# huyhoang17/DB_text_minimal

Hardware: AMD Instinct MI355X
Metric: train images/sec @640x640 bs=16/GPU (higher is better)
Workload: dtype f32

## Files before the change

### db_text_minimal_amd/csrc/winograd_wgrad_f32.hip

```cpp
#include "igemm_common.h"
#include <algorithm>

namespace {

constexpr int WG_XPX = 180, WG_XROW = 18, WG_YPX = 128, WG_YROW = 16;

struct WinoWgradParams {
    const float* x;
    const float* dy;
    float* slab;
    int N, H, W, Cx, Cy;
    int nob, nib;
    int tw, gpi, groups;
    int nsplit;
    unsigned x_bytes, dy_bytes;
    const float *x_scale, *x_shift;
};

constexpr int WL_XPX = 336, WL_YPX = 240;
template <bool LIN>
__global__ __launch_bounds__(512) __attribute__((amdgpu_waves_per_eu(2, 2))) void winograd_wgrad_f32_kernel(const WinoWgradParams p) {
    constexpr int XPX = LIN ? WL_XPX : WG_XPX, YPX = LIN ? WL_YPX : WG_YPX;
    constexpr int XCH = XPX * 16, YCH = YPX * 16;
    constexpr int NXP = (XCH + 511) / 512, NYP = (YCH + 511) / 512;
    constexpr int NBUF = LIN ? 1 : 2;
    __shared__ f32x4 smem[NBUF * (XCH + YCH)];
    const int tid = threadIdx.x, lane = tid & 63, wave = __builtin_amdgcn_readfirstlane(tid >> 6);
    const int li = lane & 31, lh = lane >> 5;
    const int irow = wave & 3, oh = wave >> 2;
    const int nsub = p.nob * p.nib;
    const int b = dbn_xcd_remap(blockIdx.x, gridDim.x);
    const int split = b / nsub, sub = b - split * nsub;
    const int ob = sub / p.nib, ib = sub - ob * p.nib;
    const int g0 = (int)((long)split * p.groups / p.nsplit), g1 = (int)((long)(split + 1) * p.groups / p.nsplit);
    const __amdgpu_buffer_rsrc_t rsX = __builtin_amdgcn_make_buffer_rsrc(const_cast<float*>(p.x), 0, p.x_bytes, 0x00020000);
    const __amdgpu_buffer_rsrc_t rsY = __builtin_amdgcn_make_buffer_rsrc(const_cast<float*>(p.dy), 0, p.dy_bytes, 0x00020000);
    const int TW = (p.W + 1) >> 1, TI = ((p.H + 1) >> 1) * TW;
    const int prow = LIN ? 2 * TW + 2 : WG_XROW, yrow = LIN ? 2 * TW : WG_YROW;
    const float rTW = 1.0f / (float)TW;

    unsigned xrel[NXP], yrel[NYP];
    int xpos[NXP], ypos[NYP];
#pragma unroll
    for (int j = 0; j < NXP; ++j) {
        const int idx = tid + j * 512, pix = idx >> 4, ch = idx & 15;
        int py, px;
        if constexpr (LIN) divmod24(pix, prow, 1.0f / (float)prow, py, px);
        else { py = pix / WG_XROW; px = pix - py * WG_XROW; }
        xrel[j] = (unsigned)((py * p.W + px) * p.Cx + ch * 4) * 4u;
        xpos[j] = idx < XCH ? (py | (px << 8)) : -1;
    }
#pragma unroll
    for (int j = 0; j < NYP; ++j) {
        const int idx = tid + j * 512, pix = idx >> 4, ch = idx & 15;
        int py, px;
        if constexpr (LIN) divmod24(pix, yrow, 1.0f / (float)yrow, py, px);
        else { py = pix >> 4; px = pix & 15; }
        yrel[j] = (unsigned)((py * p.W + px) * p.Cy + ch * 4) * 4u;
        ypos[j] = idx < YCH ? (py | (px << 8)) : -1;
    }
    f32x4 rx[NXP], ry[LIN ? 1 : NYP];
    const bool act = p.x_scale != nullptr;
    f32x4 asc_ = {0.f, 0.f, 0.f, 0.f}, ash_ = {0.f, 0.f, 0.f, 0.f};
    if (act && !LIN) {
        asc_ = *reinterpret_cast<const f32x4*>(p.x_scale + ib * 64 + (tid & 15) * 4);
        ash_ = *reinterpret_cast<const f32x4*>(p.x_shift + ib * 64 + (tid & 15) * 4);
    }
    unsigned xstatic = 0;
#pragma unroll
    for (int j = 0; j < NXP; ++j) xstatic |= (unsigned)(xpos[j] >= 0) << j;
    unsigned xvalid = 0;
    int t0 = 0, tr0 = 0;
    auto geometry = [&](int g, int& n, int& hs0, int& ws0, int& xrows) {
        n = g / p.gpi;
        const int t = g - n * p.gpi;
        if constexpr (LIN) {
            const int tfirst = t * 32, tlast = min(tfirst + 31, TI - 1);
            const int r0_ = tfirst / TW, r1_ = tlast / TW;
            hs0 = 2 * r0_ - 1;
            ws0 = -1;
            xrows = 2 * (r1_ - r0_ + 1) + 2;
        } else {
            const int ty = t / p.tw, tx = t - ty * p.tw;
            hs0 = ty * 8 - 1;
            ws0 = tx * 16 - 1;
            xrows = 10;
        }
    };
    auto load_x = [&](int g) {
        int n, hs0, ws0, xrows;
        geometry(g, n, hs0, ws0, xrows);
        const unsigned bx = (unsigned)(((n * p.H + hs0) * p.W + ws0) * p.Cx + ib * 64) * 4u;
        if (!LIN && hs0 >= 0 && hs0 + 10 <= p.H && ws0 >= 0 && ws0 + WG_XROW <= p.W) {
#pragma unroll
            for (int j = 0; j < NXP; ++j) rx[j] = buffer_load_f32x4(rsX, xpos[j] >= 0 ? bx + xrel[j] : OOB_OFFSET);
            xvalid = xstatic;
            return;
        }
#pragma unroll
        for (int j = 0; j < NXP; ++j) {
            const int py = xpos[j] & 255, px = xpos[j] >> 8;
            const bool v = xpos[j] >= 0 && py < xrows && (unsigned)(hs0 + py) < (unsigned)p.H && (unsigned)(ws0 + px) < (unsigned)p.W;
            rx[j] = buffer_load_f32x4(rsX, v ? bx + xrel[j] : OOB_OFFSET);
// ... 100 lines not shown
            float dd[4], D[4];
            auto fetch = [&](int s_) {
                const int xo = xoff2 + (2 * (s_ >> 2) * WG_XROW + 4 * (s_ & 3)) * 32, yo = yoff4 + (2 * (s_ >> 2) * WG_YROW + 4 * (s_ & 3)) * 64;
#pragma unroll
                for (int q = 0; q < 4; ++q) {
                    U1[q] = Xr1[xo + q * 32];
                    U2[q] = Xr2[xo + q * 32];
                }
                dd[0] = Yb[yo];
                dd[1] = Yb[yo + 64];
                dd[2] = Yb[yo + WG_YROW * 64];
                dd[3] = Yb[yo + WG_YROW * 64 + 64];
            };
            auto form = [&]() {
                f32x2 R[4];
#pragma unroll
                for (int q = 0; q < 4; ++q) {
                    R[q][0] = fmaf(sa, U2[q][0], U1[q][0]);
                    R[q][1] = fmaf(sa, U2[q][1], U1[q][1]);
                }
                V[0] = R[0] - R[2];
                V[1] = R[1] + R[2];
                V[2] = R[2] - R[1];
                V[3] = R[1] - R[3];
                const float r0 = fmaf(c1, dd[2], c0 * dd[0]), r1 = fmaf(c1, dd[3], c0 * dd[1]);
                D[0] = r0;
                D[1] = r0 + r1;
                D[2] = r0 - r1;
                D[3] = -r1;
            };
            fetch(0);
            form();
#pragma unroll
            for (int s = 0; s < 16; ++s) {
                f32x2 Vc[4];
                float Dc[4];
#pragma unroll
                for (int j = 0; j < 4; ++j) {
                    Vc[j] = V[j];
                    Dc[j] = D[j];
                }
                __builtin_amdgcn_sched_barrier(0);
                if (s + 1 < 16) fetch(s + 1);
                __builtin_amdgcn_sched_barrier(0);
#pragma unroll
                for (int j = 0; j < 4; ++j)
#pragma unroll
                    for (int h = 0; h < 2; ++h) acc[j][h] = __builtin_amdgcn_mfma_f32_32x32x2f32(Dc[j], Vc[j][h], acc[j][h], 0, 0, 0);
                __builtin_amdgcn_sched_barrier(0);
                if (s + 1 < 16) form();
            }
        } else {
#pragma unroll
            for (int s = 0; s < 16; ++s) {
                const int t = t0 + 2 * s + lh;
                const bool ok = t < TI;
                int ty, tx;
                divmod24(ok ? t : t0, TW, rTW, ty, tx);
                ty -= tr0;
                const int xo = (2 * ty * prow + 2 * tx) * 32, yo = (2 * ty * yrow + 2 * tx) * 64;
                const float c0s = ok ? c0 : 0.f, c1s = ok ? c1 : 0.f;
                f32x2 R[4];
#pragma unroll
                for (int q = 0; q < 4; ++q) {
                    const f32x2 u1 = Xr1[xoff2 + xo + q * 32], u2 = Xr2[xoff2 + xo + q * 32];
                    R[q][0] = fmaf(sa, u2[0], u1[0]);
                    R[q][1] = fmaf(sa, u2[1], u1[1]);
                }
                const float* const Yc = Yb + yoff4;
                const float d00 = Yc[yo], d01 = Yc[yo + 64], d10 = Yc[yo + yrow * 64], d11 = Yc[yo + yrow * 64 + 64];
                const f32x2 V[4] = {R[0] - R[2], R[1] + R[2], R[2] - R[1], R[1] - R[3]};
                const float r0 = fmaf(c1s, d10, c0s * d00), r1 = fmaf(c1s, d11, c0s * d01);
                const float D[4] = {r0, r0 + r1, r0 - r1, -r1};
#pragma unroll
                for (int j = 0; j < 4; ++j)
#pragma unroll
                    for (int h = 0; h < 2; ++h) acc[j][h] = __builtin_amdgcn_mfma_f32_32x32x2f32(D[j], V[j][h], acc[j][h], 0, 0, 0);
            }
        }
        if constexpr (!LIN) {
            if (g + 1 < g1) __syncthreads();
        }
    }
    float* const S = p.slab + ((long)b * 16 + 4 * irow) * 4096 + (oh * 32 + 4 * lh) * 64 + 2 * li;
#pragma unroll
    for (int j = 0; j < 4; ++j)
#pragma unroll
        for (int r = 0; r < 16; ++r) {
            f32x2 v;
            v[0] = acc[j][0][r];
            v[1] = acc[j][1][r];
            *reinterpret_cast<f32x2*>(S + j * 4096 + ((r & 3) + 8 * (r >> 2)) * 64) = v;
        }
}

__global__ __launch_bounds__(1024) void winograd_wgrad_reduce_serial_kernel(const float* __restrict__ slab, int nsplit, int nsub, int nib, int I,
                                                                     float* __restrict__ grad, float scale) {
    __shared__ double sh[16][64];
    __shared__ float st[576];
    const int o = blockIdx.x, ib = blockIdx.y, sub = (o >> 6) * nib + ib;
    const int pnt = threadIdx.x >> 6, il = threadIdx.x & 63;
    const float* src = slab + ((long)sub * 16 + pnt) * 4096 + (o & 63) * 64 + il;
    const long stride = (long)nsub * 16 * 4096;
    double s = 0.0;
    int z = 0;
    for (; z + 3 < nsplit; z += 4)
        s += ((double)src[z * stride] + (double)src[(z + 1) * stride]) + ((double)src[(z + 2) * stride] + (double)src[(z + 3) * stride]);
    for (; z < nsplit; ++z) s += (double)src[z * stride];
    sh[pnt][il] = s;
    __syncthreads();
    if (threadIdx.x < 576) {
        const int c = threadIdx.x / 9, tap = threadIdx.x - c * 9, r = tap / 3, q = tap - r * 3;
        auto gcol = [](int k, double v0, double v1, double v2, double v3) {
            return k == 0 ? v0 + 0.5 * (v1 + v2) : (k == 1 ? 0.5 * (v1 - v2) : 0.5 * (v1 + v2) + v3);
        };
        double t[4];
#pragma unroll
        for (int i = 0; i < 4; ++i) t[i] = gcol(q, sh[4 * i + 0][c], sh[4 * i + 1][c], sh[4 * i + 2][c], sh[4 * i + 3][c]);
        st[threadIdx.x] = (float)(gcol(r, t[0], t[1], t[2], t[3]) * (double)scale);
    }
    __syncthreads();
    const int n = min(64, I - ib * 64) * 9;
    float* dst = grad + ((long)o * I + ib * 64) * 9;
    for (int k = threadIdx.x; k < n; k += 1024) dst[k] = st[k];
}

template <int ZL>
__global__ __launch_bounds__(256) void winograd_wgrad_reduce_kernel(const float* __restrict__ slab, int nsplit, int nsub, int nib, int I,
                                                                    float* __restrict__ grad, float scale) {
    constexpr int OG = 32 / ZL, ZH = ZL / 2;
    __shared__ double part[ZH * OG][16][32 + 1];
    __shared__ double sh[OG][16][32];
    __shared__ float st[OG * 288];
    const int ib = blockIdx.y >> 1, ih = blockIdx.y & 1;
    const int iq = threadIdx.x & 7, og = (threadIdx.x >> 3) % OG, zl2 = threadIdx.x / (8 * OG), zl = zl2 % ZH;
    const int o = blockIdx.x * OG + og, sub = (o >> 6) * nib + ib;
    const float* src = slab + (long)sub * 16 * 4096 + (o & 63) * 64 + ih * 32 + iq * 4;
    const long stride = (long)nsub * 16 * 4096;
    const int z0 = (int)((long)zl2 * nsplit / ZL), z1 = (int)((long)(zl2 + 1) * nsplit / ZL);
    double acc[16][4];
#pragma unroll
    for (int pt = 0; pt < 16; ++pt)
#pragma unroll
        for (int e = 0; e < 4; ++e) acc[pt][e] = 0.0;
    for (int z = z0; z < z1; ++z) {
        f32x4 v[16];
#pragma unroll
        for (int pt = 0; pt < 16; ++pt) v[pt] = *reinterpret_cast<const f32x4*>(src + z * stride + pt * 4096);
#pragma unroll
        for (int pt = 0; pt < 16; ++pt)
#pragma unroll
            for (int e = 0; e < 4; ++e) acc[pt][e] += (double)v[pt][e];
    }
    if (zl2 >= ZH) {
#pragma unroll
        for (int pt = 0; pt < 16; ++pt)
#pragma unroll
            for (int e = 0; e < 4; ++e) part[zl * OG + og][pt][iq * 4 + e] = acc[pt][e];
    }
    __syncthreads();
    if (zl2 < ZH) {
#pragma unroll
        for (int pt = 0; pt < 16; ++pt)
#pragma unroll
            for (int e = 0; e < 4; ++e) part[zl * OG + og][pt][iq * 4 + e] += acc[pt][e];
    }
    __syncthreads();
    for (int k = threadIdx.x; k < OG * 16 * 32; k += 256) {
        const int g = k >> 9, pt = (k >> 5) & 15, c = k & 31;
        double s_ = 0.0;
#pragma unroll
        for (int q = 0; q < ZH; ++q) s_ += part[q * OG + g][pt][c];
        sh[g][pt][c] = s_;
    }
    __syncthreads();
    for (int k = threadIdx.x; k < OG * 288; k += 256) {
        const int g = k / 288, kk = k - g * 288, c = kk / 9, tap = kk - c * 9, r = tap / 3, q = tap - r * 3;
        auto gcol = [](int w, double v0, double v1, double v2, double v3) {
            return w == 0 ? v0 + 0.5 * (v1 + v2) : (w == 1 ? 0.5 * (v1 - v2) : 0.5 * (v1 + v2) + v3);
        };
        double t[4];
#pragma unroll
        for (int i = 0; i < 4; ++i) t[i] = gcol(q, sh[g][4 * i + 0][c], sh[g][4 * i + 1][c], sh[g][4 * i + 2][c], sh[g][4 * i + 3][c]);
        st[k] = (float)(gcol(r, t[0], t[1], t[2], t[3]) * (double)scale);
    }
    __syncthreads();
    const int c0 = ib * 64 + ih * 32;
    const int n = max(0, min(32, I - c0)) * 9;
    for (int k = threadIdx.x; k < OG * n; k += 256) {
        const int g = k / n, kk = k - g * n;
        grad[((long)(blockIdx.x * OG + g) * I + c0) * 9 + kk] = st[g * 288 + kk];
    }
}

int wwg_splits(int groups, int nsub) {
    static const int wgs = dbn_env_int("DBN_WWG_WGS", 256);
    int ns = std::max(1, wgs / nsub);
    return std::min(ns, groups);
}

bool wwg_linear_fits(int H, int W) {
    const int TW = (W + 1) / 2, TH = (H + 1) / 2;
    const int R = std::min(TH, (30 + TW) / TW + 1);
    return (2 * R + 2) * (2 * TW + 2) <= WL_XPX && 2 * R * 2 * TW <= WL_YPX;
}
double wwg_fill(int H, int W, bool lin) {
    if (lin) {
        const long TI = (long)((H + 1) / 2) * ((W + 1) / 2);
        return (double)TI / (double)((TI + 31) / 32 * 32);
    }
    return (double)H * W / ((double)((H + 7) / 8 * 8) * ((W + 15) / 16 * 16));
}
bool wwg_linear(int H, int W) {
    static const int env = dbn_env_int("DBN_WWG_LIN", 1);
    return env && wwg_linear_fits(H, W) && wwg_fill(H, W, true) > wwg_fill(H, W, false) + 0.2;
}
int wwg_groups(int N, int H, int W) {
    if (wwg_linear(H, W)) return N * (int)(((long)((H + 1) / 2) * ((W + 1) / 2) + 31) / 32);
    return N * ((H + 7) / 8) * ((W + 15) / 16);
}
bool wwg_wide(int nsplit) { return nsplit >= 128; }

}

extern "C" {

int dbn_winograd_wgrad_eligible(int N, int H, int W, int O, int Cb, int I) {
    if (N < 1 || H < 1 || W < 1 || O % 64 || Cb % 64 || I < 1 || I > Cb) return 0;
    const long px = (long)N * H * W;
    if (px * std::max(O, Cb) * 4 >= dbn_g_byte_limit) return 0;
    return wwg_fill(H, W, wwg_linear(H, W)) >= 0.5;
}
int dbn_winograd_wgrad_linear(int H, int W) { return wwg_linear(H, W); }
long dbn_winograd_wgrad_slab_floats(int N, int H, int W, int O, int Cb) {
    const int nsub = (O / 64) * (Cb / 64);
    return (long)wwg_splits(wwg_groups(N, H, W), nsub) * nsub * 16 * 4096;
}
int dbn_winograd_wgrad_f32(int phases, const float* dy, const float* x, const float* x_scale, const float* x_shift, float* slab, float* grad,
                           int N, int H, int W, int O, int Cb, int I, float scale, void* stream) {
    DBN_REQUIRE(dy && x && slab && grad && phases >= 1 && phases <= 3 && !x_scale == !x_shift);
    DBN_REQUIRE(dbn_winograd_wgrad_eligible(N, H, W, O, Cb, I));
    WinoWgradParams p;
    p.x = x;
    p.dy = dy;
    p.slab = slab;
    p.x_scale = x_scale;
    p.x_shift = x_shift;
    p.N = N;
    p.H = H;
    p.W = W;
    p.Cx = Cb;
    p.Cy = O;
    p.nob = O / 64;
    p.nib = Cb / 64;
    const bool lin = wwg_linear(H, W);
    p.tw = (W + 15) / 16;
    p.groups = wwg_groups(N, H, W);
    p.gpi = p.groups / N;
    p.nsplit = wwg_splits(p.groups, p.nob * p.nib);
    p.x_bytes = (unsigned)((long)N * H * W * Cb * 4);
    p.dy_bytes = (unsigned)((long)N * H * W * O * 4);
    hipStream_t st = (hipStream_t)stream;
    if (phases & 1) {
        const dim3 grid(p.nsplit * p.nob * p.nib);
        if (lin) hipLaunchKernelGGL(winograd_wgrad_f32_kernel<true>, grid, dim3(512), 0, st, p);
        else hipLaunchKernelGGL(winograd_wgrad_f32_kernel<false>, grid, dim3(512), 0, st, p);
    }
    if (phases & 2) {
        const int nsub = p.nob * p.nib;
        if (wwg_wide(p.nsplit))
            hipLaunchKernelGGL(winograd_wgrad_reduce_kernel<32>, dim3(O, 2 * p.nib), dim3(256), 0, st, slab, p.nsplit, nsub, p.nib, I, grad, scale);
        else
            hipLaunchKernelGGL(winograd_wgrad_reduce_serial_kernel, dim3(O, p.nib), dim3(1024), 0, st, slab, p.nsplit, nsub, p.nib, I, grad, scale);
    }
    return dbn_status();
}

int dbn_winograd_describe(int N, int H, int W, int O, int Cb, void* plan) {
    DBN_REQUIRE(plan && N > 0 && H > 0 && W > 0 && O > 0 && O % 64 == 0 && Cb > 0 && Cb % 64 == 0);
    dbn_winograd_plan* const q = reinterpret_cast<dbn_winograd_plan*>(plan);
    q->fwd_lin = dbn_winograd_linear(H, W);
    q->fwd_rows = dbn_winograd_rows(N, H, W);
    q->wgrad_lin = wwg_linear(H, W);
    q->wgrad_groups = wwg_groups(N, H, W);
    q->wgrad_nsub = (O / 64) * (Cb / 64);
    q->wgrad_nsplit = wwg_splits(q->wgrad_groups, q->wgrad_nsub);
    q->wgrad_wide = wwg_wide(q->wgrad_nsplit);
    return DBN_OK;
}

}
```

### db_text_minimal_amd/engine.py

```python
import contextlib
import ctypes
import os

import torch

from . import _lib
from ._lib import check

DEAD_PREFIXES = ('backbone.fc.', 'backbone.smooth.')
K_STEP_DEFAULT = 50.0


def _p(t):
    return None if t is None else t.data_ptr()


def _out_hw(conv, H, W):
    k, s, p = conv.k, conv.stride, conv.padding
    return (H + 2 * p - k) // s + 1, (W + 2 * p - k) // s + 1


NO_BN = (None, None, 0.0, 0.0) + (None, ) * 7


# ... 646 lines not shown
        if self.L.dbn_igemm_kernel_config(at, self.ns, 2, N, H, W, C, 2 * H, 2 * W, Co, 2, 2, 2, 0, 0, 1) & 32:
            self.prof.begin('convt2x2_f32_kernel<%d>' % C, flops, 0.0, 'convT fwd ' + name)
        else:
            self._prof_igemm(N * 4 * H * W, Co, flops, 'convT fwd ' + name, 2)

    def _prof_igemm(self, M, Cd, flops, tag='', mode=0, geom=None, epi=0):
        cfg = self.L.dbn_igemm_tile_config_ns(M, Cd, self.ns)
        at = 3 if self._use_planes else self.at
        if geom is not None and mode < 2:
            N, Hs, Ws, Cs, Hd, Wd, R, stride, pad = geom
            ks = self.L.dbn_igemm_splitk_plan_ns(N * Hd * Wd, Cd, R * R * Cs, Cs, self.ns) if self.splitk else 1
            cfg = self.L.dbn_igemm_kernel_config(at, self.ns, mode, N, Hs, Ws, Cs, Hd, Wd, Cd, R, R, stride, pad, 0, ks)
        blk = 'false' if (geom is not None and mode == 0 and geom[3] % 16 != 0) else 'true'
        nbytes = 0.0
        if geom is not None:
            N, Hs, Ws, Cs, Hd, Wd = geom[:6]
            nbytes = float(N) * (Hs * Ws * Cs + Hd * Wd * Cd) * (4 if self.at == 0 else 2)
        if geom is not None and mode < 2 and geom[6] == 3 and geom[7] == 1 and geom[8] == 1 and self.ns == 1 and \
                self.L.dbn_wres16_would_run(at, mode, geom[0], geom[4], geom[5], geom[3], Cd, epi, 0):
            self.prof.begin('conv3x3_wres16_kernel<%d,%d,%d,%d>' % (at, geom[3], Cd, mode), flops, nbytes, tag)
            return
        label = IGEMM_TILE_NAMES[cfg & 15] % (mode, self.ns, at, 'true' if cfg & 16 else 'false', epi, blk)
        if (cfg & 15) == 1 and at in (1, 2) and self.ns == 1:
            label = label.replace('<128,128,2,2,', '<128,128,1,4,')
        self.prof.begin(label, flops, nbytes, tag)

    def _winograd_dgrad(self, name, dy, conv, dx, accumulate, consumer, panel=None):
        N, H, W, O = dy.shape
        Cd = dx.shape[3]
        up = panel if panel is not None else self._winograd_panel(name, conv.weight, O, dgrad=1)
        L = self.L
        rows = L.dbn_winograd_rows(N, H, W)
        a = dict(y=None, zmask=None, msc=None, msh=None, mean=None, rstd=None, part=None, y2=None, mean2=None, rstd2=None, part2=None)
        if consumer is not None:
            bn_name, y, zmask = consumer[:3]
            second = consumer[3] if len(consumer) > 3 else None
            assert tuple(y.shape) == (N, H, W, Cd) and (zmask is None or zmask.shape == y.shape), (name, bn_name)
            a.update(y=y, zmask=zmask, mean=self.bufs[bn_name + '/mean'], rstd=self.bufs[bn_name + '/rstd'],
                     part=self.fbuf(bn_name + '/bnb_part', 2 * Cd * rows))
            if zmask is None:
                a.update(msc=self.bufs[bn_name + '/scale'], msh=self.bufs[bn_name + '/shift'])
            if second is not None:
                assert zmask is not None and second[1].shape == y.shape
                a.update(y2=second[1], mean2=self.bufs[second[0] + '/mean'], rstd2=self.bufs[second[0] + '/rstd'],
                         part2=self.fbuf(second[0] + '/bnb_part', 2 * Cd * rows))
        if self.prof:
            extra = sum(a[k] is not None for k in ('y', 'zmask', 'y2')) + int(bool(accumulate))
            self.prof.begin('winograd_f32_kernel', 2.0 * N * H * W * O * Cd * 4, 4.0 * N * H * W * (O + Cd * (1 + extra)), 'dgrad ' + name)
        check(L.dbn_winograd_dgrad_bnsums_f32(dy.data_ptr(), up.data_ptr(), dx.data_ptr(), N, H, W, O, Cd, int(accumulate), _p(a['y']),
                                              _p(a['zmask']), _p(a['msc']), _p(a['msh']), _p(a['mean']), _p(a['rstd']), _p(a['part']),
                                              _p(a['y2']), _p(a['mean2']), _p(a['rstd2']), _p(a['part2']), None, self.stream),
              'winograd dgrad ' + name)
        if self.prof:
            self.prof.end()
        if consumer is not None:
            self._bnb_sums[consumer[0]] = (a['part'], rows)
            if len(consumer) > 3 and consumer[3] is not None:
                self._bnb_sums[consumer[3][0]] = (a['part2'], rows)

    def conv_dgrad(self, name, dy, conv, dx, accumulate, version=None, consumer=None):
        N, Ho, Wo, O = dy.shape
        _, H, W, I = dx.shape
        if (version is None and self.winograd and self.ns == 0 and self.at == 0 and conv.k == 3 and conv.stride == 1 and conv.padding == 1
                and (Ho, Wo) == (H, W) and dy.dtype == torch.float32 and I == conv.cin and O == conv.cout
                and bool(self.L.dbn_winograd_eligible(N, H, W, O, I))):
            if consumer is not None and not (self.fuse_bn_bwd_sums and not (self.prof is not None and self.prof.labels is None and not self.prof_fused)):
                consumer = None
            self._winograd_dgrad(name, dy, conv, dx, accumulate, consumer)
            return
        wpk = self.pack(name, conv.weight, 1, conv.stride, version=version)
        args = (dy.data_ptr(), wpk.data_ptr(), None, dx.data_ptr(), N, Ho, Wo, O, H, W, I, conv.k, conv.k, conv.stride, conv.padding, 1,
                int(accumulate), 0)
        if consumer is not None and not self._bnb_eligible(args):
            consumer = None
        if self.prof:
            self._prof_igemm(N * H * W, I, 2.0 * N * Ho * Wo * O * I * conv.k * conv.k, 'dgrad ' + name, 2 if conv.stride == 2 else 1,
                             (N, Ho, Wo, O, H, W, conv.k, conv.stride, conv.padding), epi=int(consumer is not None))
        self._igemm('igemm dgrad ' + name, *args, consumer=consumer)
        if self.prof:
            self.prof.end()

    defer_wgrad_reduce = False
    winograd_wgrad = True

    def wgrad(self, name, sm, big, O, I, k, stride, pad, gview, defer=False, big_act=None):
        N, Ho, Wo, _ = sm.shape
        _, H, W, Cb = big.shape
        if ((k, stride, pad) == (3, 1, 1) and (Ho, Wo) == (H, W)
                and self.plan(_VirtualConv(I, O, k, stride, pad, None, None), big.shape, True,
                              fp32_tensors=sm.dtype == torch.float32 and big.dtype == torch.float32).winograd_wgrad):
            slab = self.scratch('_wgrad_slab', self.L.dbn_winograd_wgrad_slab_floats(N, H, W, O, Cb))
            asc, ash = (big_act[0].data_ptr(), big_act[1].data_ptr()) if big_act is not None else (None, None)
            wargs = (sm.data_ptr(), big.data_ptr(), asc, ash, slab.data_ptr(), gview.data_ptr(), N, H, W, O, Cb, I, self.grad_scale, self.stream)
            if self.prof:
                self.prof.begin('winograd_wgrad_f32_kernel', 2.0 * N * ((H + 1) // 2) * ((W + 1) // 2) * 16 * O * Cb, 0.0, 'wgrad ' + name)
                check(self.L.dbn_winograd_wgrad_f32(1, *wargs), 'winograd wgrad ' + name)
                self.prof.end()
                self.prof.begin('wgrad_reduce_kernel', 0.0, 0.0, 'wgrad reduce ' + name)
                check(self.L.dbn_winograd_wgrad_f32(2, *wargs), 'winograd wgrad reduce ' + name)
                self.prof.end()
            else:
                check(self.L.dbn_winograd_wgrad_f32(3, *wargs), 'winograd wgrad ' + name)
            return
        assert big_act is None, name
        defer = defer and self.defer_wgrad_reduce and self.prof is None and Cb % 64 == 0
        slab = self.scratch('_wgrad_slab/' + name if defer else '_wgrad_slab',
                            self.L.dbn_wgrad_slab_floats_hw(N, Ho, Wo, O, H, W, Cb, k, k, 4 if self.at == 0 else 2))
        at, smp, bigp = self.at, sm.data_ptr(), big.data_ptr()
        if self._use_planes and sm.dtype == torch.float32 and big.dtype == torch.float32:
            at, smp, bigp = 3, self._planes(sm).data_ptr(), self._planes(big).data_ptr()
        args = (at, self.ns, smp, bigp, slab.data_ptr(), gview.data_ptr(), N, Ho, Wo, O, H, W, Cb, I, k, k, stride,
                pad, self.grad_scale, self.stream)
        if self.prof:
            cfg = self.L.dbn_wgrad_kernel_config_hw(at, self.ns, O, Cb, k, k, stride, pad, Ho, Wo, H, W)
            wname = WGRAD_TILE_NAMES[cfg & 15] % (self.ns, at, (cfg >> 6) & 1)
            if cfg & 32:
                wname = 'wgrad_patch_kernel<%d,%d>' % (self.ns, at)
            elif cfg & 16:
                wname = 'wgrad_tr_kernel<' + wname.split('<')[1].rsplit(',', 3)[0] + '>'
            self.prof.begin(wname,
                            2.0 * N * Ho * Wo * O * I * k * k, 0.0, 'wgrad ' + name)
            check(self.L.dbn_wgrad_phase_t(1, *args), 'wgrad ' + name)
            self.prof.end()
            self.prof.begin('wgrad_reduce_kernel', 0.0, 0.0, 'wgrad reduce ' + name)
            check(self.L.dbn_wgrad_phase_t(2, *args), 'wgrad reduce ' + name)
            self.prof.end()
        elif defer:
            check(self.L.dbn_wgrad_phase_t(1, *args), 'wgrad ' + name)
            key = (name, args[:-1])
            job = self._reduce_job_cache.get(key)
            if job is None:
                job = _lib.WgradReduceJob()
                check(self.L.dbn_wgrad_reduce_describe(*args[:-1], ctypes.byref(job)), 'wgrad reduce describe ' + name)
                self._reduce_job_cache[key] = job
            self._reduce_pending.append((key, job))
        else:
            check(self.L.dbn_wgrad_t(*args), 'wgrad ' + name)

    def flush_wgrad_reduces(self):
        self._flush_wgrads()
        if not self._reduce_pending:
            return
        pending, self._reduce_pending = self._reduce_pending, []
        sig = tuple(k for k, _ in pending)
        ent = self._reduce_tables.get(sig)
        if ent is None:
            arr = (_lib.WgradReduceJob * len(pending))(*[j for _, j in pending])
            first = [0]
            for _, j in pending:
                first.append(first[-1] + j.blocks)
            ent = (self._device_table(arr), torch.tensor(first, dtype=torch.int32, device=self.flat.device),
                   len(pending), first[-1], max(j.smem_bytes for _, j in pending))
            self._reduce_tables[sig] = ent
        table, first, n, blocks, smem = ent
        with self.side_stream():
            check(self.L.dbn_wgrad_reduce_many(table.data_ptr(), first.data_ptr(), n, blocks, smem, self.stream), 'wgrad_reduce_many')

    def _flush_wgrads(self):
        if self._wgrad_fifo:
            fifo, self._wgrad_fifo = self._wgrad_fifo, []
            for fn in fifo:
                fn()

    def conv_wgrad(self, name, dy, x, conv, x_act=None):
        self._presplit(dy, x)

        def launch():
            with self.side_stream():
                self.wgrad(name, dy, x, conv.cout, conv.cin, conv.k, conv.stride, conv.padding, self.grad_views[name + '.weight'], defer=True,
                           big_act=x_act)
                if conv.bias is not None and name + '.bias' not in self._bias_done:
                    self.col_sum(dy, self.grad_views[name + '.bias'])
        late = self.at != 0
        if late and self.overlap_wgrad and not self._in_side and self.prof is None:
            self._wgrad_fifo.append(launch)
        else:
            launch()

    def convT_fwd(self, name, x, ct, out_name):
        got = self._convt16(name, x, ct, out_name)
        if got is not None:
            return got[0]
        N, H, W, C = x.shape
        wpk = self.pack(name, ct.weight, 1, 2)
        y = self.buf(out_name, N, 2 * H, 2 * W, ct.cout)
# ... 968 lines not shown
```

### include/dbnet_hip.h

```cpp
#ifndef DBNET_HIP_H
#define DBNET_HIP_H
#ifdef __cplusplus
extern "C" {
#endif


int dbn_pack_weights(const float* w_oihw, int O, int I, int R, int S, int mode, int stride, float* out, void* stream);
long dbn_igemm_panel_floats(int O, int I, int R, int S, int mode, int stride);
int dbn_igemm_packed_floats(int K, int Cd);

int dbn_igemm_f32(const float* src, const float* wpk, const float* bias, float* dst, int N, int Hs, int Ws, int Cs, int Hd,
                  int Wd, int Cd, int R, int S, int stride, int pad, int mode, int accumulate, int tile_hint, void* stream);

int dbn_pack_weights_bf16s(const float* w_oihw, int O, int I, int R, int S, int mode, int stride, int ns, float* out, void* stream);
typedef struct dbn_pack_job {
    const float* w;
    void* out;
    int O, I, R, S, mode, Cs, Cd, f;
} dbn_pack_job;
int dbn_pack_weights_batched(const void* jobs, int n, int ns, void* stream);
long dbn_igemm_bf16s_panel_floats(int O, int I, int R, int S, int mode, int stride, int ns);
int dbn_igemm_bf16s(const float* src, const float* wpk, const float* bias, float* dst, int N, int Hs, int Ws, int Cs, int Hd,
                    int Wd, int Cd, int R, int S, int stride, int pad, int mode, int accumulate, int tile_hint, int ns,
                    void* stream);
// ... 62 lines not shown
                              int H, int W, int Cs, int Cd, void* stream);
int dbn_pyramid_conv_act_t(int first_level, int at, const void* s0, const void* s1, const void* s2, const void* s3, const float* w0,
                           const float* w1, const float* w2, const float* w3, const float* bias, int relu, void* dst, int N, int H, int W,
                           int Cs, int Cd, int ns, void* stream);
int dbn_bn_eval_coef(int C, const float* gamma, const float* beta, const float* run_mean, const float* run_var, float eps,
                     float* scale, float* shift, void* stream);
int dbn_bn_apply(const float* y, const float* scale, const float* shift, const float* res, const float* res_scale,
                 const float* res_shift, float* out, long M, int C, int relu, void* stream);
int dbn_bn_backward(const float* y, const float* zmask, const float* mask_scale, const float* mask_shift, const float* dout,
                    const float* save_mean, const float* save_rstd,
                    const float* gamma, float* dy, float* gout, int gout_accumulate, float* dgamma, float* dbeta, int M, int C,
                    float grad_scale, float* ws, void* stream);
int dbn_bn_backward_from_sums(const float* sums, const float* y, const float* zmask, const float* mask_scale, const float* mask_shift,
                              const float* dout, const float* save_mean, const float* save_rstd, const float* gamma, float* dy,
                              float* gout, int gout_accumulate, float* dgamma, float* dbeta, int M, int C, float grad_scale,
                              float* ws, void* stream);
int dbn_bn_backward_ex(const float* sums, const float* y, const float* zmask, const float* mask_scale, const float* mask_shift,
                       const float* dout, const float* save_mean, const float* save_rstd, const float* gamma, float* dy, float* gout,
                       int gout_accumulate, float* dgamma, float* dbeta, float* dbias_conv, int M, int C, float grad_scale, float* ws,
                       void* stream);
int dbn_col_sum(const float* x, int M, int C, float* out, float scale, float* ws, void* stream);

int dbn_bnrelu_maxpool_fwd(const float* y, const float* scale, const float* shift, float* out, int N, int H, int W, int C,
                           void* stream);
int dbn_bnrelu_maxpool_bwd(const float* y, const float* scale, const float* shift, const float* pooled, const float* dpool,
                           float* dz, int N, int H, int W, int C, void* stream);

int dbn_nearest_up_fwd(const float* src, const float* addend, float* dst, int N, int Hs, int Ws, int C, int H, int W, int Cdst,
                       int coff, void* stream);
int dbn_nearest_up_bwd(const float* dbig, float* dsrc, int N, int Hs, int Ws, int C, int H, int W, int Cbig, int coff,
                       int accumulate, void* stream);

int dbn_bilinear_fwd(const float* src, float* dst, long planes, int Hs, int Ws, int H, int W, void* stream);
int dbn_bilinear_bwd(const float* ddst, float* dsrc, long planes, int Hs, int Ws, int H, int W, void* stream);

int dbn_fpn_combine_weights(const float* w, int Co, int Cin, int group, int Cg, float* wd, void* stream);
int dbn_fpn_scatter_wgrad(const float* t0, const float* t1, const float* t2, const float* t3, int Co, int Cg, float* dw,
                          void* stream);

int dbn_nchw3_to_nhwc4(const float* x, float* out, int N, int H, int W, void* stream);
int dbn_add_inplace(const float* x, float* y, long n, void* stream);

int dbn_head_tail_fwd(const float* xb, const float* xt, const float* wb, const float* wt, const float* bias_b,
                      const float* bias_t, const float* bn_scale_b, const float* bn_shift_b, const float* bn_scale_t,
                      const float* bn_shift_t, float* out, int N, int Hq, int Wq, int channels, float kstep, void* stream);
int dbn_head_tail_bwd_ws_floats(void);
int dbn_head_tail_bwd(const float* xb, const float* xt, const float* wb, const float* wt, const float* preds,
                      const float* dpreds, const float* bn_scale_b, const float* bn_shift_b, const float* bn_scale_t,
                      const float* bn_shift_t, const float* bn_mean_b, const float* bn_rstd_b, const float* bn_mean_t,
                      const float* bn_rstd_t, float* bn_sums, float* dxb, float* dxt, float* dw_b, float* dbias_b, float* dw_t,
                      float* dbias_t, int N, int Hq, int Wq, int channels, float kstep, float grad_scale, float* ws, void* stream);

int dbn_set_winograd_persistent(int on);
int dbn_set_winograd_stagger(int permille);
int dbn_set_winograd_blocks_per_barrier(int n);
int dbn_winograd_eligible(int N, int H, int W, int Cs, int Cd);
long dbn_winograd_panel_floats(int O, int Cs);
int dbn_winograd_pack(const float* w_oihw, int O, int I, int Cs, int dgrad, float* out, void* stream);
typedef struct dbn_winograd_pack_job {
    const float* w;
    float* out;
    int O, I, Cs, dgrad;
} dbn_winograd_pack_job;
int dbn_winograd_pack_batched(const void* jobs, int n, void* stream);
int dbn_winograd_rows(int N, int H, int W);
int dbn_winograd_dgrad_bnsums_f32(const float* dy, const float* upanel, float* dx, int N, int H, int W, int Cs, int Cd, int accumulate,
                                  const void* y, const void* zmask, const float* mask_scale, const float* mask_shift,
                                  const float* save_mean, const float* save_rstd, float* part, const void* y2, const float* save_mean2,
                                  const float* save_rstd2, float* part2, const dbn_bnb_final* fin, void* stream);
long dbn_winograd_ws_floats(int N, int H, int W, int Cd);
int dbn_winograd_conv_bn_act_f32(const float* src, const float* in_scale, const float* in_shift, const float* upanel, const float* bias,
                                 float* dst, int N, int H, int W, int Cs, int Cd, const float* gamma, const float* beta, float eps,
                                 float momentum, float* run_mean, float* run_var, float* scale, float* shift, float* save_mean,
                                 float* save_rstd, float* ws, void* stream);
int dbn_winograd_conv_bn_f32(const float* src, const float* upanel, const float* bias, float* dst, int N, int H, int W, int Cs, int Cd,
                             const float* gamma, const float* beta, float eps, float momentum, float* run_mean, float* run_var,
                             float* scale, float* shift, float* save_mean, float* save_rstd, float* ws, void* stream);

int dbn_winograd_wgrad_eligible(int N, int H, int W, int O, int Cb, int I);
int dbn_winograd_wgrad_linear(int H, int W);
long dbn_winograd_wgrad_slab_floats(int N, int H, int W, int O, int Cb);
int dbn_winograd_wgrad_f32(int phases, const float* dy, const float* x, const float* x_scale, const float* x_shift, float* slab, float* grad,
                           int N, int H, int W, int O, int Cb, int I, float scale, void* stream);
typedef struct dbn_winograd_plan {
    int fwd_lin, fwd_rows;
    int wgrad_lin, wgrad_groups, wgrad_nsub, wgrad_nsplit, wgrad_wide;
} dbn_winograd_plan;
int dbn_winograd_describe(int N, int H, int W, int O, int Cb, void* plan);

int dbn_db_loss_ws_bytes(void);
int dbn_db_loss_fwd(const float* preds, const float* gts, int N, int H, int W, int channels, float alpha, float beta,
                    double negative_ratio, float eps, float* losses, float* coef, void* ws, void* stream);
int dbn_db_loss_bwd(const float* preds, const float* gts, const float* coef, const float* grad_losses, float alpha, float beta,
                    int N, int H, int W, int channels, float* dpreds, void* stream);
int dbn_db_loss_sum_fwd(const float* preds, const float* gts, int N, int H, int W, int channels, float alpha, float beta,
                        double negative_ratio, float eps, float* losses, float* coef, void* ws, void* stream);
int dbn_db_loss_frac_fwd(const float* preds, const float* gts, int N, int H, int W, int channels, float alpha, float beta,
                         double negative_ratio, float eps, int sum, float* losses, float* coef, void* ws, void* stream);

long dbn_db_loss_ohem_ws_bytes(int N, int H, int W);
int dbn_db_loss_ohem_fwd(const float* preds, const float* gts, int N, int H, int W, int channels, float alpha, float beta,
                         double negative_ratio, float eps, float* losses, float* coef, void* ws, void* stream);
int dbn_db_loss_ohem_bwd(const float* preds, const float* gts, const float* coef, const float* grad_losses, const void* ws,
                         float alpha, float beta, int N, int H, int W, int channels, float* dpreds, void* stream);

int dbn_pixel_confusion(const float* preds, long batch_stride, const float* gt, const float* mask, int N, int H, int W, float thresh,
                        double* hist, void* stream);

int dbn_adam_step(float* p, const float* g, float* m, float* v, long n, float lr, float beta1, float beta2, float eps, int step,
                  float grad_scale, void* stream);

int dbn_grad_accumulate(float* acc, const float* g, long n, int first, void* stream);
long dbn_grad_sqnorm_ws_doubles(long n);
int dbn_grad_sqnorm(const float* g, long n, double* partials, double* out, void* stream);
int dbn_adam_step_ex(float* p, const float* g, float* m, float* v, float* vmax, long n, float lr, float beta1, float beta2, float eps,
                     float weight_decay, int step, float grad_scale, const double* sqnorm, float max_norm, void* stream);

int dbn_optim_max_groups(void);
int dbn_optim_max_runs(void);
int dbn_sgd_step(float* p, const float* g, float* buf, long n, const float* lr, const float* weight_decay, int ngroups, const int* run_end,
                 const int* run_group, int nruns, float momentum, float dampening, int nesterov, int first, float grad_scale,
                 const double* sqnorm, float max_norm, float* shadow, float ema_decay, float ema_one_minus, void* stream);
int dbn_adamw_step(float* p, const float* g, float* m, float* v, float* vmax, long n, const float* lr, const float* weight_decay, int ngroups,
                   const int* run_end, const int* run_group, int nruns, float beta1, float beta2, float eps, int decoupled, int step,
                   float grad_scale, const double* sqnorm, float max_norm, float* shadow, float ema_decay, float ema_one_minus,
                   void* stream);

int dbn_has_experiments(void);

int dbn_clock_probe(void* out2, int microseconds, void* stream);
int dbn_wall_clock_khz(void);

int dbn_deform_im2col(const float* x, const float* offset, float* cols, int N, int H, int W, int C, int Ho, int Wo, int R, int S,
                      int stride, int pad, int off_stride, void* stream);
long dbn_deform_col2im_ws_bytes(int N, int H, int W, int C, int Ho, int Wo, int R, int S);
int dbn_deform_col2im(const float* dcols, const float* x, const float* offset, float* dx, float* doffset, int accumulate, void* ws, int N,
                      int H, int W, int C, int Ho, int Wo, int R, int S, int stride, int pad, int off_stride, void* stream);
int dbn_permute_weight(const float* src, float* dst, int O, int C, int T, int to_ohwi, float scale, void* stream);

int dbn_binarize_u8(const float* pred, int N, int channels, int H, int W, float thresh, unsigned char* out, void* stream);
int dbn_box_scores(const float* bitmap, int H, int W, const float* boxes, int K, int P, float* scores, void* stream);

int dbn_gt_maps(const double* verts, const double* dist, const int* meta, const int* img_off, const int* ixy, int N, int P, int S,
                int max_verts, int max_off_pts, float scale, float tmin, float* out, void* stream);
int dbn_normalize_u8(const unsigned char* in, int N, int H, int W, float m0, float m1, float m2, float* out, void* stream);
int dbn_poly_offset(const double* xy, int n, const double* delta, int* out_xy, int cap, int* out_n);
int dbn_poly_offset_paths(const double* xy, int n, const double* delta, int* out_xy, int cap, int* out_n, int* out_paths);

int dbn_warp_affine_u8(const unsigned char* src, long src_bytes, const long long* desc, const double* coef, int N, int max_h, int max_w,
                       unsigned char* dst, long dst_bytes, void* stream);
int dbn_resize_cubic_u8(const unsigned char* src, long src_bytes, const long long* desc, const double* coef, int N, int max_h, int max_w,
                        unsigned char* dst, long dst_bytes, void* stream);
int dbn_resize_linear_norm_u8(const unsigned char* src, long src_bytes, const long long* desc, const double* coef, int N, int CH, int CW,
                              float m0, float m1, float m2, float* out, void* stream);

int dbn_perspective_maps(const float* quads, int K, int out_h, int out_w, double* fwd, double* inv);
int dbn_warp_perspective_u8(const unsigned char* src, long src_bytes, const long long* desc, const double* inv, int K, int out_h, int out_w,
                            unsigned char* dst, long dst_bytes, void* stream);

int dbn_polygon_ribbons(const double* xy, const long long* offs, int K, int segments, int half, int threads, int* knots,
                        unsigned char* valid, int* ends, double* info);
int dbn_polygon_ribbons_device(const double* xy, const long long* offs, int K, long total_vertices, int segments, int half, int* knots,
                               unsigned char* valid, int* ends, double* info, void* stream);
int dbn_rectify_u8(const unsigned char* src, long src_bytes, const long long* desc, const int* knots, const unsigned char* valid, int K,
                   int segments, int out_h, int out_w, unsigned char* dst, long dst_bytes, void* stream);

// ... 248 lines not shown
```

Before: 737.6.

## Apply Winograd output transform in wgrad kernel, store 9 taps instead of 16

The wgrad MFMA kernel now applies the 4x4-to-3x3 Winograd weight-gradient transform itself before writing partials. It does the column pass in registers and the row pass through an LDS exchange between waves. The slab then holds 9 taps per split instead of 16 points, which cuts slab write and reduce read traffic by about 44% and removes the transform from the reduce kernels. The costs are extra LDS round trips and syncthreads in the wgrad epilogue, plus float32 rather than double precision for the per-split transform.

```diff
diff --git a/db_text_minimal_amd/csrc/winograd_wgrad_f32.hip b/db_text_minimal_amd/csrc/winograd_wgrad_f32.hip
--- a/db_text_minimal_amd/csrc/winograd_wgrad_f32.hip
+++ b/db_text_minimal_amd/csrc/winograd_wgrad_f32.hip
@@ -18,7 +18,11 @@
 };
 
 constexpr int WL_XPX = 336, WL_YPX = 240;
-template <bool LIN>
+template <typename T>
+__device__ __forceinline__ T wwg_gcol(int k, T v0, T v1, T v2, T v3) {
+    return k == 0 ? v0 + (T)0.5 * (v1 + v2) : (k == 1 ? (T)0.5 * (v1 - v2) : (T)0.5 * (v1 + v2) + v3);
+}
+template <bool LIN, bool TAPS>
 __global__ __launch_bounds__(512) __attribute__((amdgpu_waves_per_eu(2, 2))) void winograd_wgrad_f32_kernel(const WinoWgradParams p) {
     constexpr int XPX = LIN ? WL_XPX : WG_XPX, YPX = LIN ? WL_YPX : WG_YPX;
     constexpr int XCH = XPX * 16, YCH = YPX * 16;
@@ -285,109 +289,159 @@
             if (g + 1 < g1) __syncthreads();
         }
     }
-    float* const S = p.slab + ((long)b * 16 + 4 * irow) * 4096 + (oh * 32 + 4 * lh) * 64 + 2 * li;
-#pragma unroll
-    for (int j = 0; j < 4; ++j)
-#pragma unroll
-        for (int r = 0; r < 16; ++r) {
-            f32x2 v;
-            v[0] = acc[j][0][r];
-            v[1] = acc[j][1][r];
-            *reinterpret_cast<f32x2*>(S + j * 4096 + ((r & 3) + 8 * (r >> 2)) * 64) = v;
-        }
-}
-
-__global__ __launch_bounds__(1024) void winograd_wgrad_reduce_serial_kernel(const float* __restrict__ slab, int nsplit, int nsub, int nib, int I,
-                                                                     float* __restrict__ grad, float scale) {
-    __shared__ double sh[16][64];
+    if constexpr (TAPS) {
+#pragma unroll
+        for (int h = 0; h < 2; ++h)
+#pragma unroll
+            for (int r = 0; r < 16; ++r) {
+                const float u0 = acc[0][h][r], u1 = acc[1][h][r], u2 = acc[2][h][r], u3 = acc[3][h][r];
+                acc[0][h][r] = wwg_gcol(0, u0, u1, u2, u3);
+                acc[1][h][r] = wwg_gcol(1, u0, u1, u2, u3);
+                acc[2][h][r] = wwg_gcol(2, u0, u1, u2, u3);
+            }
+        constexpr int WV = 48 * 64;
+        static_assert(8 * WV * 4 <= (int)sizeof(smem), "the exchange of a round must fit the staging LDS");
+        float* const ex = reinterpret_cast<float*>(smem);
+        float* const mine = ex + wave * WV + lane;
+        const float* const theirs = ex + oh * 4 * WV + lane;
+        float* const S = p.slab + (long)b * 9 * 4096 + (oh * 32 + 4 * lh + 2 * (irow & 1) + 8 * (irow >> 1)) * 64 + 2 * li;
+#pragma unroll
+        for (int rd = 0; rd < 2; ++rd) {
+            __syncthreads();
+#pragma unroll
+            for (int q = 0; q < 3; ++q)
+#pragma unroll
+                for (int h = 0; h < 2; ++h)
+#pragma unroll
+                    for (int e = 0; e < 8; ++e) mine[((q * 2 + h) * 8 + e) * 64] = acc[q][h][8 * rd + e];
+            __syncthreads();
+#pragma unroll
+            for (int q = 0; q < 3; ++q)
+#pragma unroll
+                for (int e = 0; e < 2; ++e) {
+                    f32x2 c[4];
+#pragma unroll
+                    for (int i = 0; i < 4; ++i)
+#pragma unroll
+                        for (int h = 0; h < 2; ++h) c[i][h] = theirs[i * WV + ((q * 2 + h) * 8 + 2 * irow + e) * 64];
+#pragma unroll
+                    for (int t = 0; t < 3; ++t) {
+                        f32x2 v;
+                        v[0] = wwg_gcol(t, c[0][0], c[1][0], c[2][0], c[3][0]);
+                        v[1] = wwg_gcol(t, c[0][1], c[1][1], c[2][1], c[3][1]);
+                        *reinterpret_cast<f32x2*>(S + (t * 3 + q) * 4096 + (16 * rd + e) * 64) = v;
+                    }
+                }
+        }
+    } else {
+        float* const S = p.slab + ((long)b * 16 + 4 * irow) * 4096 + (oh * 32 + 4 * lh) * 64 + 2 * li;
+#pragma unroll
+        for (int j = 0; j < 4; ++j)
+#pragma unroll
+            for (int r = 0; r < 16; ++r) {
+                f32x2 v;
+                v[0] = acc[j][0][r];
+                v[1] = acc[j][1][r];
+                *reinterpret_cast<f32x2*>(S + j * 4096 + ((r & 3) + 8 * (r >> 2)) * 64) = v;
+            }
+    }
+}
+
+template <int NP>
+__global__ __launch_bounds__(NP * 64) void winograd_wgrad_reduce_serial_kernel(const float* __restrict__ slab, int nsplit, int nsub, int nib, int I,
+                                                                          float* __restrict__ grad, float scale) {
+    static_assert(NP == 16 || NP == 9, "16 points or 9 taps");
+    __shared__ double sh[NP == 16 ? 16 : 1][64];
     __shared__ float st[576];
     const int o = blockIdx.x, ib = blockIdx.y, sub = (o >> 6) * nib + ib;
     const int pnt = threadIdx.x >> 6, il = threadIdx.x & 63;
-    const float* src = slab + ((long)sub * 16 + pnt) * 4096 + (o & 63) * 64 + il;
-    const long stride = (long)nsub * 16 * 4096;
+    const float* src = slab + ((long)sub * NP + pnt) * 4096 + (o & 63) * 64 + il;
+    const long stride = (long)nsub * NP * 4096;
     double s = 0.0;
     int z = 0;
     for (; z + 3 < nsplit; z += 4)
         s += ((double)src[z * stride] + (double)src[(z + 1) * stride]) + ((double)src[(z + 2) * stride] + (double)src[(z + 3) * stride]);
     for (; z < nsplit; ++z) s += (double)src[z * stride];
-    sh[pnt][il] = s;
-    __syncthreads();
-    if (threadIdx.x < 576) {
-        const int c = threadIdx.x / 9, tap = threadIdx.x - c * 9, r = tap / 3, q = tap - r * 3;
-        auto gcol = [](int k, double v0, double v1, double v2, double v3) {
-            return k == 0 ? v0 + 0.5 * (v1 + v2) : (k == 1 ? 0.5 * (v1 - v2) : 0.5 * (v1 + v2) + v3);
-        };
-        double t[4];
-#pragma unroll
-        for (int i = 0; i < 4; ++i) t[i] = gcol(q, sh[4 * i + 0][c], sh[4 * i + 1][c], sh[4 * i + 2][c], sh[4 * i + 3][c]);
-        st[threadIdx.x] = (float)(gcol(r, t[0], t[1], t[2], t[3]) * (double)scale);
+    if constexpr (NP == 16) {
+        sh[pnt][il] = s;
+        __syncthreads();
+        if (threadIdx.x < 576) {
+            const int c = threadIdx.x / 9, tap = threadIdx.x - c * 9, r = tap / 3, q = tap - r * 3;
+            double t[4];
+#pragma unroll
+            for (int i = 0; i < 4; ++i) t[i] = wwg_gcol(q, sh[4 * i + 0][c], sh[4 * i + 1][c], sh[4 * i + 2][c], sh[4 * i + 3][c]);
+            st[threadIdx.x] = (float)(wwg_gcol(r, t[0], t[1], t[2], t[3]) * (double)scale);
+        }
+    } else {
+        st[il * 9 + pnt] = (float)(s * (double)scale);
     }
     __syncthreads();
     const int n = min(64, I - ib * 64) * 9;
     float* dst = grad + ((long)o * I + ib * 64) * 9;
-    for (int k = threadIdx.x; k < n; k += 1024) dst[k] = st[k];
-}
-
-template <int ZL>
+    for (int k = threadIdx.x; k < n; k += NP * 64) dst[k] = st[k];
+}
+
+template <int ZL, int NP>
 __global__ __launch_bounds__(256) void winograd_wgrad_reduce_kernel(const float* __restrict__ slab, int nsplit, int nsub, int nib, int I,
                                                                     float* __restrict__ grad, float scale) {
+    static_assert(NP == 16 || NP == 9, "16 points or 9 taps");
     constexpr int OG = 32 / ZL, ZH = ZL / 2;
-    __shared__ double part[ZH * OG][16][32 + 1];
-    __shared__ double sh[OG][16][32];
+    __shared__ double part[ZH * OG][NP][32 + 1];
+    __shared__ double sh[NP == 16 ? OG : 1][NP][32];
     __shared__ float st[OG * 288];
     const int ib = blockIdx.y >> 1, ih = blockIdx.y & 1;
     const int iq = threadIdx.x & 7, og = (threadIdx.x >> 3) % OG, zl2 = threadIdx.x / (8 * OG), zl = zl2 % ZH;
     const int o = blockIdx.x * OG + og, sub = (o >> 6) * nib + ib;
-    const float* src = slab + (long)sub * 16 * 4096 + (o & 63) * 64 + ih * 32 + iq * 4;
-    const long stride = (long)nsub * 16 * 4096;
+    const float* src = slab + (long)sub * NP * 4096 + (o & 63) * 64 + ih * 32 + iq * 4;
+    const long stride = (long)nsub * NP * 4096;
     const int z0 = (int)((long)zl2 * nsplit / ZL), z1 = (int)((long)(zl2 + 1) * nsplit / ZL);
-    double acc[16][4];
-#pragma unroll
-    for (int pt = 0; pt < 16; ++pt)
+    double acc[NP][4];
+#pragma unroll
+    for (int pt = 0; pt < NP; ++pt)
 #pragma unroll
         for (int e = 0; e < 4; ++e) acc[pt][e] = 0.0;
     for (int z = z0; z < z1; ++z) {
-        f32x4 v[16];
-#pragma unroll
-        for (int pt = 0; pt < 16; ++pt) v[pt] = *reinterpret_cast<const f32x4*>(src + z * stride + pt * 4096);
-#pragma unroll
-        for (int pt = 0; pt < 16; ++pt)
+        f32x4 v[NP];
+#pragma unroll
+        for (int pt = 0; pt < NP; ++pt) v[pt] = *reinterpret_cast<const f32x4*>(src + z * stride + pt * 4096);
+#pragma unroll
+        for (int pt = 0; pt < NP; ++pt)
 #pragma unroll
             for (int e = 0; e < 4; ++e) acc[pt][e] += (double)v[pt][e];
     }
     if (zl2 >= ZH) {
 #pragma unroll
-        for (int pt = 0; pt < 16; ++pt)
+        for (int pt = 0; pt < NP; ++pt)
 #pragma unroll
             for (int e = 0; e < 4; ++e) part[zl * OG + og][pt][iq * 4 + e] = acc[pt][e];
     }
     __syncthreads();
     if (zl2 < ZH) {
 #pragma unroll
-        for (int pt = 0; pt < 16; ++pt)
+        for (int pt = 0; pt < NP; ++pt)
 #pragma unroll
             for (int e = 0; e < 4; ++e) part[zl * OG + og][pt][iq * 4 + e] += acc[pt][e];
     }
     __syncthreads();
-    for (int k = threadIdx.x; k < OG * 16 * 32; k += 256) {
-        const int g = k >> 9, pt = (k >> 5) & 15, c = k & 31;
+    for (int k = threadIdx.x; k < OG * NP * 32; k += 256) {
+        const int g = k / (NP * 32), pt = (k >> 5) % NP, c = k & 31;
         double s_ = 0.0;
 #pragma unroll
         for (int q = 0; q < ZH; ++q) s_ += part[q * OG + g][pt][c];
-        sh[g][pt][c] = s_;
+        if constexpr (NP == 16) sh[g][pt][c] = s_;
+        else st[g * 288 + c * 9 + pt] = (float)(s_ * (double)scale);
     }
     __syncthreads();
-    for (int k = threadIdx.x; k < OG * 288; k += 256) {
-        const int g = k / 288, kk = k - g * 288, c = kk / 9, tap = kk - c * 9, r = tap / 3, q = tap - r * 3;
-        auto gcol = [](int w, double v0, double v1, double v2, double v3) {
-            return w == 0 ? v0 + 0.5 * (v1 + v2) : (w == 1 ? 0.5 * (v1 - v2) : 0.5 * (v1 + v2) + v3);
-        };
-        double t[4];
-#pragma unroll
-        for (int i = 0; i < 4; ++i) t[i] = gcol(q, sh[g][4 * i + 0][c], sh[g][4 * i + 1][c], sh[g][4 * i + 2][c], sh[g][4 * i + 3][c]);
-        st[k] = (float)(gcol(r, t[0], t[1], t[2], t[3]) * (double)scale);
-    }
-    __syncthreads();
+    if constexpr (NP == 16) {
+        for (int k = threadIdx.x; k < OG * 288; k += 256) {
+            const int g = k / 288, kk = k - g * 288, c = kk / 9, tap = kk - c * 9, r = tap / 3, q = tap - r * 3;
+            double t[4];
+#pragma unroll
+            for (int i = 0; i < 4; ++i) t[i] = wwg_gcol(q, sh[g][4 * i + 0][c], sh[g][4 * i + 1][c], sh[g][4 * i + 2][c], sh[g][4 * i + 3][c]);
+            st[k] = (float)(wwg_gcol(r, t[0], t[1], t[2], t[3]) * (double)scale);
+        }
+        __syncthreads();
+    }
     const int c0 = ib * 64 + ih * 32;
     const int n = max(0, min(32, I - c0)) * 9;
     for (int k = threadIdx.x; k < OG * n; k += 256) {
@@ -422,7 +476,14 @@
     if (wwg_linear(H, W)) return N * (int)(((long)((H + 1) / 2) * ((W + 1) / 2) + 31) / 32);
     return N * ((H + 7) / 8) * ((W + 15) / 16);
 }
-bool wwg_wide(int nsplit) { return nsplit >= 128; }
+bool wwg_wide(int nsplit, bool taps) {
+    static const int from = dbn_env_int("DBN_WWG_TAPS_WIDE", 128);
+    return nsplit >= (taps ? from : 128);
+}
+long wwg_slab_floats(int N, int H, int W, int O, int Cb, bool taps) {
+    const int nsub = (O / 64) * (Cb / 64);
+    return (long)wwg_splits(wwg_groups(N, H, W), nsub) * nsub * (taps ? 9 : 16) * 4096;
+}
 
 }
 
@@ -435,12 +496,10 @@
     return wwg_fill(H, W, wwg_linear(H, W)) >= 0.5;
 }
 int dbn_winograd_wgrad_linear(int H, int W) { return wwg_linear(H, W); }
-long dbn_winograd_wgrad_slab_floats(int N, int H, int W, int O, int Cb) {
-    const int nsub = (O / 64) * (Cb / 64);
-    return (long)wwg_splits(wwg_groups(N, H, W), nsub) * nsub * 16 * 4096;
-}
-int dbn_winograd_wgrad_f32(int phases, const float* dy, const float* x, const float* x_scale, const float* x_shift, float* slab, float* grad,
-                           int N, int H, int W, int O, int Cb, int I, float scale, void* stream) {
+long dbn_winograd_wgrad_slab_floats(int N, int H, int W, int O, int Cb) { return wwg_slab_floats(N, H, W, O, Cb, false); }
+long dbn_winograd_wgrad_taps_slab_floats(int N, int H, int W, int O, int Cb) { return wwg_slab_floats(N, H, W, O, Cb, true); }
+static int wwg_run(bool taps, int phases, const float* dy, const float* x, const float* x_scale, const float* x_shift, float* slab, float* grad,
+                   int N, int H, int W, int O, int Cb, int I, float scale, void* stream) {
     DBN_REQUIRE(dy && x && slab && grad && phases >= 1 && phases <= 3 && !x_scale == !x_shift);
     DBN_REQUIRE(dbn_winograd_wgrad_eligible(N, H, W, O, Cb, I));
     WinoWgradParams p;
@@ -466,20 +525,23 @@
     hipStream_t st = (hipStream_t)stream;
     if (phases & 1) {
         const dim3 grid(p.nsplit * p.nob * p.nib);
-        if (lin) hipLaunchKernelGGL(winograd_wgrad_f32_kernel<true>, grid, dim3(512), 0, st, p);
-        else hipLaunchKernelGGL(winograd_wgrad_f32_kernel<false>, grid, dim3(512), 0, st, p);
+        auto* const kern = lin ? (taps ? winograd_wgrad_f32_kernel<true, true> : winograd_wgrad_f32_kernel<true, false>)
+                               : (taps ? winograd_wgrad_f32_kernel<false, true> : winograd_wgrad_f32_kernel<false, false>);
+        hipLaunchKernelGGL(kern, grid, dim3(512), 0, st, p);
     }
     if (phases & 2) {
         const int nsub = p.nob * p.nib;
-        if (wwg_wide(p.nsplit))
-            hipLaunchKernelGGL(winograd_wgrad_reduce_kernel<32>, dim3(O, 2 * p.nib), dim3(256), 0, st, slab, p.nsplit, nsub, p.nib, I, grad, scale);
-        else
-            hipLaunchKernelGGL(winograd_wgrad_reduce_serial_kernel, dim3(O, p.nib), dim3(1024), 0, st, slab, p.nsplit, nsub, p.nib, I, grad, scale);
+        if (wwg_wide(p.nsplit, taps)) {
+            auto* const kern = taps ? winograd_wgrad_reduce_kernel<32, 9> : winograd_wgrad_reduce_kernel<32, 16>;
+            hipLaunchKernelGGL(kern, dim3(O, 2 * p.nib), dim3(256), 0, st, slab, p.nsplit, nsub, p.nib, I, grad, scale);
+        } else {
+            auto* const kern = taps ? winograd_wgrad_reduce_serial_kernel<9> : winograd_wgrad_reduce_serial_kernel<16>;
+            hipLaunchKernelGGL(kern, dim3(O, p.nib), dim3(taps ? 576 : 1024), 0, st, slab, p.nsplit, nsub, p.nib, I, grad, scale);
+        }
     }
     return dbn_status();
 }
-
-int dbn_winograd_describe(int N, int H, int W, int O, int Cb, void* plan) {
+static int wwg_describe(bool taps, int N, int H, int W, int O, int Cb, void* plan) {
     DBN_REQUIRE(plan && N > 0 && H > 0 && W > 0 && O > 0 && O % 64 == 0 && Cb > 0 && Cb % 64 == 0);
     dbn_winograd_plan* const q = reinterpret_cast<dbn_winograd_plan*>(plan);
     q->fwd_lin = dbn_winograd_linear(H, W);
@@ -488,8 +550,19 @@
     q->wgrad_groups = wwg_groups(N, H, W);
     q->wgrad_nsub = (O / 64) * (Cb / 64);
     q->wgrad_nsplit = wwg_splits(q->wgrad_groups, q->wgrad_nsub);
-    q->wgrad_wide = wwg_wide(q->wgrad_nsplit);
+    q->wgrad_wide = wwg_wide(q->wgrad_nsplit, taps);
     return DBN_OK;
 }
-
-}
+int dbn_winograd_wgrad_f32(int phases, const float* dy, const float* x, const float* x_scale, const float* x_shift, float* slab, float* grad,
+                           int N, int H, int W, int O, int Cb, int I, float scale, void* stream) {
+    return wwg_run(false, phases, dy, x, x_scale, x_shift, slab, grad, N, H, W, O, Cb, I, scale, stream);
+}
+int dbn_winograd_wgrad_taps_f32(int phases, const float* dy, const float* x, const float* x_scale, const float* x_shift, float* slab, float* grad,
+                                int N, int H, int W, int O, int Cb, int I, float scale, void* stream) {
+    return wwg_run(true, phases, dy, x, x_scale, x_shift, slab, grad, N, H, W, O, Cb, I, scale, stream);
+}
+
+int dbn_winograd_describe(int N, int H, int W, int O, int Cb, void* plan) { return wwg_describe(false, N, H, W, O, Cb, plan); }
+int dbn_winograd_wgrad_taps_describe(int N, int H, int W, int O, int Cb, void* plan) { return wwg_describe(true, N, H, W, O, Cb, plan); }
+
+}
diff --git a/db_text_minimal_amd/engine.py b/db_text_minimal_amd/engine.py
--- a/db_text_minimal_amd/engine.py
+++ b/db_text_minimal_amd/engine.py
@@ -752,6 +752,7 @@
 
     defer_wgrad_reduce = False
     winograd_wgrad = True
+    winograd_wgrad_taps = True
 
     def wgrad(self, name, sm, big, O, I, k, stride, pad, gview, defer=False, big_act=None):
         N, Ho, Wo, _ = sm.shape
@@ -759,18 +760,20 @@
         if ((k, stride, pad) == (3, 1, 1) and (Ho, Wo) == (H, W)
                 and self.plan(_VirtualConv(I, O, k, stride, pad, None, None), big.shape, True,
                               fp32_tensors=sm.dtype == torch.float32 and big.dtype == torch.float32).winograd_wgrad):
-            slab = self.scratch('_wgrad_slab', self.L.dbn_winograd_wgrad_slab_floats(N, H, W, O, Cb))
+            run, slab_floats = ((self.L.dbn_winograd_wgrad_taps_f32, self.L.dbn_winograd_wgrad_taps_slab_floats) if self.winograd_wgrad_taps else
+                                (self.L.dbn_winograd_wgrad_f32, self.L.dbn_winograd_wgrad_slab_floats))
+            slab = self.scratch('_wgrad_slab', slab_floats(N, H, W, O, Cb))
             asc, ash = (big_act[0].data_ptr(), big_act[1].data_ptr()) if big_act is not None else (None, None)
             wargs = (sm.data_ptr(), big.data_ptr(), asc, ash, slab.data_ptr(), gview.data_ptr(), N, H, W, O, Cb, I, self.grad_scale, self.stream)
             if self.prof:
                 self.prof.begin('winograd_wgrad_f32_kernel', 2.0 * N * ((H + 1) // 2) * ((W + 1) // 2) * 16 * O * Cb, 0.0, 'wgrad ' + name)
-                check(self.L.dbn_winograd_wgrad_f32(1, *wargs), 'winograd wgrad ' + name)
+                check(run(1, *wargs), 'winograd wgrad ' + name)
                 self.prof.end()
                 self.prof.begin('wgrad_reduce_kernel', 0.0, 0.0, 'wgrad reduce ' + name)
-                check(self.L.dbn_winograd_wgrad_f32(2, *wargs), 'winograd wgrad reduce ' + name)
+                check(run(2, *wargs), 'winograd wgrad reduce ' + name)
                 self.prof.end()
             else:
-                check(self.L.dbn_winograd_wgrad_f32(3, *wargs), 'winograd wgrad ' + name)
+                check(run(3, *wargs), 'winograd wgrad ' + name)
             return
         assert big_act is None, name
         defer = defer and self.defer_wgrad_reduce and self.prof is None and Cb % 64 == 0
diff --git a/include/dbnet_hip.h b/include/dbnet_hip.h
--- a/include/dbnet_hip.h
+++ b/include/dbnet_hip.h
@@ -168,6 +168,10 @@
 long dbn_winograd_wgrad_slab_floats(int N, int H, int W, int O, int Cb);
 int dbn_winograd_wgrad_f32(int phases, const float* dy, const float* x, const float* x_scale, const float* x_shift, float* slab, float* grad,
                            int N, int H, int W, int O, int Cb, int I, float scale, void* stream);
+long dbn_winograd_wgrad_taps_slab_floats(int N, int H, int W, int O, int Cb);
+int dbn_winograd_wgrad_taps_f32(int phases, const float* dy, const float* x, const float* x_scale, const float* x_shift, float* slab,
+                                float* grad, int N, int H, int W, int O, int Cb, int I, float scale, void* stream);
+int dbn_winograd_wgrad_taps_describe(int N, int H, int W, int O, int Cb, void* plan);
 typedef struct dbn_winograd_plan {
     int fwd_lin, fwd_rows;
     int wgrad_lin, wgrad_groups, wgrad_nsub, wgrad_nsplit, wgrad_wide;
```

New measurement: 740.2, median of 6. Within noise of the previous version (+0.4%).
